# linhthi/BLISS-GNN

Measured on AMD Instinct MI355X. Metric: steps/sec (train step: sample_blocks + gather + SAGE fwd/bwd + Adam + exp3), reddit-like, higher is better.
Workload: dtype bf16

## Files before the change

bliss_gnn_amd/_lib.py:

```python
import ctypes as C
import os

_HERE = os.path.dirname(os.path.abspath(__file__))
LIB_PATH = os.path.join(_HERE, "libbliss_gnn.so")

EINVAL = -1
MODE_BANDIT, MODE_LADIES, MODE_UNIFORM_NODES, MODE_PARTIALS = 0, 1, 4, 8

ERR_BITS = {
    1: "frontier larger than 2^31-1 edges",
    2: "candidate capacity exceeded / seed id out of range",
    4: "kept-node capacity exceeded",
    8: "block-edge capacity exceeded",
    16: "non-finite or negative weight reached an exact reduction",
    32: "exact sum left its fixed-point range",
    64: "seed capacity exceeded",
    128: "random stream ran short / generator made no progress",
    256: "a cross-stream flag never came (bliss_flag_wait timed out)",
}


class Graph(C.Structure):
    _fields_ = [("indptr", C.c_void_p), ("indices", C.c_void_p), ("eid", C.c_void_p),
                ("num_nodes", C.c_int32), ("num_edges", C.c_int64)]


class NodeMaps(C.Structure):
    _fields_ = [("local_id", C.c_void_p), ("first_pos", C.c_void_p), ("acc_p2", C.c_void_p)]


class LayerCounts(C.Structure):
    _fields_ = [("S", C.c_int32), ("E", C.c_int32), ("C", C.c_int32), ("K", C.c_int32), ("B", C.c_int32),
                ("err", C.c_int32), ("iters", C.c_int32), ("all_one", C.c_int32), ("c", C.c_double)]


class LayerWs(C.Structure):
    _fields_ = [("counts", C.c_void_p), ("seg_ptr", C.c_void_p), ("seed_acc", C.c_void_p), ("chunk_cnt", C.c_void_p),
                ("cand_nid", C.c_void_p), ("p", C.c_void_p), ("P", C.c_void_p), ("new_id", C.c_void_p),
                ("kept_nid", C.c_void_p), ("node_prob", C.c_void_p), ("hist", C.c_void_p), ("src_cnt", C.c_void_p), ("cap_c", C.c_int32), ("cap_k", C.c_int32),
                ("n_bins", C.c_int32), ("bin_cap", C.c_int64), ("bin_cursor", C.c_void_p), ("bin_rec", C.c_void_p),
                ("bitmap", C.c_void_p), ("word_prefix", C.c_void_p), ("touched_key", C.c_void_p), ("touched_sum", C.c_void_p),
                ("span_seg", C.c_void_p), ("kept_rec", C.c_void_p), ("span_cnt", C.c_void_p), ("kept_rec_positions", C.c_int64),
                ("kept_map", C.c_void_p), ("entry_flag", C.c_void_p),
                ("fs_ticket", C.c_void_p), ("fs_fanout", C.c_int32), ("fs_is_last", C.c_int32), ("fs_rng_cap", C.c_int32),
                ("fs_reserved", C.c_int32), ("fs_eps", C.c_double), ("fs_rng_ctl", C.c_void_p), ("fs_layer_off", C.c_void_p),
                ("block_ready_flag", C.c_void_p)]


class Exp3Block(C.Structure):
    _fields_ = [("w_pos", C.c_void_p), ("row_sum", C.c_void_p), ("scratch", C.c_void_p), ("norm_out", C.c_void_p),
                ("blk_indptr", C.c_void_p), ("blk_src", C.c_void_p), ("blk_dst", C.c_void_p), ("blk_pos", C.c_void_p),
                ("q_ij", C.c_void_p), ("node_prob", C.c_void_p), ("embed_norm", C.c_void_p), ("alpha_or_null", C.c_void_p),
                ("dst_nid", C.c_void_p), ("n_edges_dev", C.c_void_p), ("rewards_out", C.c_void_p), ("edges_bound", C.c_int32)]


EXP3_MAX_BLOCKS = 8


class Exp3RankLists(C.Structure):
    _fields_ = [("w_pos", C.c_void_p * EXP3_MAX_BLOCKS), ("row_sum", C.c_void_p * EXP3_MAX_BLOCKS),
                ("pos_off_words", C.c_int32 * EXP3_MAX_BLOCKS), ("factor_off_bf16", C.c_int32 * EXP3_MAX_BLOCKS),
                ("count_off_words", C.c_int32 * EXP3_MAX_BLOCKS), ("bound", C.c_int32 * EXP3_MAX_BLOCKS),
                ("n_blocks", C.c_int32), ("n_ranks", C.c_int32), ("rank_stride_words", C.c_int64)]


class PackLists(C.Structure):
    _fields_ = [("pos", C.c_void_p * EXP3_MAX_BLOCKS), ("n_dev", C.c_void_p * EXP3_MAX_BLOCKS),
                ("pos_off_words", C.c_int32 * EXP3_MAX_BLOCKS), ("count_off_words", C.c_int32 * EXP3_MAX_BLOCKS),
                ("bound", C.c_int32 * EXP3_MAX_BLOCKS), ("n_blocks", C.c_int32)]


class TileGemm(C.Structure):
    _fields_ = [("a1", C.c_void_p), ("a1_stride", C.c_int64), ("ids", C.c_void_p),
                ("w1", C.c_void_p), ("w1_stride", C.c_int64), ("k1", C.c_int32),
                ("a2", C.c_void_p), ("a2_stride", C.c_int64), ("w2", C.c_void_p), ("w2_stride", C.c_int64), ("k2", C.c_int32),
                ("bias", C.c_void_p), ("m_bound", C.c_int32), ("m_dev", C.c_void_p), ("n", C.c_int32),
                ("out", C.c_void_p), ("out_stride", C.c_int64), ("a_copy", C.c_void_p), ("copy_stride", C.c_int64),
                ("in_norm", C.c_void_p), ("out_norm", C.c_void_p),
                ("relu", C.c_int32), ("drop_p", C.c_float), ("drop_seed", C.c_uint32), ("drop_ctr", C.c_void_p)]


class DGrad(C.Structure):
    _fields_ = [("a1", C.c_void_p), ("a1_stride", C.c_int64), ("w1", C.c_void_p), ("w1_stride", C.c_int64), ("k1", C.c_int32),
                ("a2", C.c_void_p), ("a2_stride", C.c_int64), ("w2", C.c_void_p), ("w2_stride", C.c_int64), ("k2", C.c_int32),
                ("m2_bound", C.c_int32), ("m2_dev", C.c_void_p),
                ("m_bound", C.c_int32), ("m_dev", C.c_void_p), ("n", C.c_int32), ("out", C.c_void_p), ("out_stride", C.c_int64)]


class WGrad(C.Structure):
    _fields_ = [("d", C.c_void_p), ("d_stride", C.c_int64), ("n_out", C.c_int32),
                ("x", C.c_void_p), ("x_stride", C.c_int64), ("k_in", C.c_int32),
                ("rows_bound", C.c_int32), ("rows_dev", C.c_void_p),
                ("dw", C.c_void_p), ("dw_stride", C.c_int64), ("db", C.c_void_p)]


class GatFused(C.Structure):
    _fields_ = [("indptr", C.c_void_p), ("src", C.c_void_p), ("n_dst", C.c_int32), ("n_dst_dev", C.c_void_p),
                ("feat", C.c_void_p), ("feat_stride", C.c_int64), ("attn", C.c_void_p), ("heads", C.c_int32), ("head_dim", C.c_int32),
                ("negative_slope", C.c_float), ("e", C.c_void_p), ("a", C.c_void_p), ("a_drop", C.c_void_p),
                ("rst", C.c_void_p), ("rst_stride", C.c_int64),
                ("drop_p", C.c_float), ("drop_seed", C.c_uint32), ("drop_ctr", C.c_void_p), ("drop_ctr_used", C.c_void_p),
                ("g", C.c_void_p), ("g_stride", C.c_int64), ("de", C.c_void_p), ("d_er", C.c_void_p), ("d_er_stride", C.c_int64),
                ("dattn_part", C.c_void_p),
                ("wg_row", C.c_void_p), ("n_wg_dev", C.c_void_p), ("cap_wg", C.c_int32), ("row_ws", C.c_void_p), ("seg_part", C.c_void_p),
                ("err", C.c_void_p)]


ADAM_MAX_TENSORS = 32


class AdamTensors(C.Structure):
    _fields_ = [("param", C.c_void_p * ADAM_MAX_TENSORS), ("grad", C.c_void_p * ADAM_MAX_TENSORS),
                ("exp_avg", C.c_void_p * ADAM_MAX_TENSORS), ("exp_avg_sq", C.c_void_p * ADAM_MAX_TENSORS),
                ("numel", C.c_int64 * ADAM_MAX_TENSORS), ("count", C.c_int32)]


class BlockOut(C.Structure):
    _fields_ = [("indptr", C.c_void_p), ("src", C.c_void_p), ("dst", C.c_void_p), ("pos", C.c_void_p),
                ("eid", C.c_void_p), ("edge_weights", C.c_void_p), ("q_ij", C.c_void_p), ("t_indptr", C.c_void_p),
                ("t_edge", C.c_void_p), ("t_scratch", C.c_void_p), ("cap_b", C.c_int32)]


_P, _I32, _I64, _F, _D = C.c_void_p, C.c_int32, C.c_int64, C.c_float, C.c_double

SIGNATURES = {
    "bliss_layer_counts_bytes": [],
    "bliss_frontier_prob": [C.POINTER(Graph), C.POINTER(NodeMaps), _P, _P, _I32, _P, _I32, C.c_int, _F, _F, _I64, C.POINTER(LayerWs), _P],
    "bliss_rng_stream_begin": [_P, _P, _P, _P, _I32, _P],
    "bliss_rng_stream_wait": [_P, _P, _P, C.c_int, _I32, _P],
    "bliss_rng_stream_end": [_P, _P, _P, _I32, _P, _P],
    "bliss_rng_stream_chain": [_P, _P, _P, _P, _I32, _P, _I32, _P, _P],
    "bliss_rng_stream_ready": [_P],
    "bliss_rng_prepare": [_I32, _P],
    "bliss_mt_jump_poly": [_I64, _P],
    "bliss_flag_wait": [_P, _P, _P],
    "bliss_flag_set_spin_bound": [C.c_int64],
    "bliss_flag_raise": [_P, _P],
    "bliss_gather_rows": [_P, _I64, _P, _I32, _I32, _P, _I64, _P, _P],
    "bliss_exp3_apply_ranks": [C.POINTER(Exp3RankLists), _P, _P, _P, _P],
    "bliss_pack_lists": [C.POINTER(PackLists), _P, _P],
    "bliss_mt19937_uniform": [_P, _P, _I32, _P, _I32, _P],
    "bliss_poisson_select": [C.POINTER(LayerWs), _I32, _D, _P, _P, _P, C.c_int, _I32, _I64, _P],
    "bliss_multinomial_select": [C.POINTER(LayerWs), _P, _I32, _P],
    "bliss_tile_gemm": [C.POINTER(TileGemm), C.POINTER(TileGemm), _P],
    "bliss_cross_entropy": [_P, _I64, _P, _I32, _I32, _P, _P, _I64, _P, _P, _P, _P],
    "bliss_cross_entropy_sum": [_P, _I64, _P, _I64, _P, _P, _I32, _I32, _P, _P, _I64, _P, _P, _P, _P],
    "bliss_cross_entropy_masked": [_P, _I64, _P, _I64, _P, _I32, _P, _I32, _I32, _P, _F, _I32, _P, _P, _I64, _P, _P, _P, _P],
    "bliss_bce_logits": [_P, _I64, _P, _I32, _I32, _P, _P, _I64, _P, _P, _P, _P],
    "bliss_bce_logits_sum": [_P, _I64, _P, _I64, _P, _P, _I32, _I32, _P, _P, _I64, _P, _P, _P, _P],
    "bliss_bce_logits_masked": [_P, _I64, _P, _I64, _P, _I32, _P, _I32, _I32, _P, _F, _I32, _P, _P, _I64, _P, _P, _P, _P],
    "bliss_adam_step": [C.POINTER(AdamTensors), _P, _F, _F, _F, _F, _P],
    "bliss_cand_importance": [_P, _I32, C.c_int, _P, _P, _P],
    "bliss_poisson_scale": [_P, _P, _I32, _D, _P, _P],
    "bliss_keyed_select": [_P, _P, _P, _I32, _P, C.c_uint64, C.c_uint64, _I32, _P, _P, _P],
    "bliss_exp3_normalize_global": [_P, _I64, _P, _P, _P, _P, _P],
    "bliss_build_block": [C.POINTER(Graph), C.POINTER(NodeMaps), _P, _P, _I32, C.c_int, _F, _F, _I64, C.POINTER(LayerWs), C.POINTER(BlockOut), _P],
    "bliss_normalized_edata": [C.POINTER(Graph), _P, _P],
    "bliss_embed_norm": [_P, _I32, _I32, _I64, _P, _P],
    "bliss_spmm_fwd": [_P, _P, _P, _P, _P, _I64, _I32, _P, _I32, _I32, C.c_int, _P, _I64, C.c_int, _P, _P],
    "bliss_spmm_bwd": [_P, _P, _P, _P, _P, _P, _P, _I64, _I32, _P, _I32, _I32, C.c_int, _P, _I64, C.c_int, _P, _P],
    "bliss_block_transpose": [_P, _P, _I32, _I32, _I32, _P, _P, _P, _I64, _P],
    "bliss_spmm_chunk_edges": [_I32],
    "bliss_sage_epilogue_fwd": [_P, _I64, _P, _I64, _I32, _I32, _F, C.c_uint32, _P, _P, _I64, _P, _P],
    "bliss_sage_epilogue_bwd": [_P, _I64, _P, _I64, _I32, _I32, _F, _P, _I64, _P],
    "bliss_gat_chunk_edges": [],
    "bliss_graph_prepare": [_P, _P, _I64, _I32, C.c_int, _P, _P, _P, _P, _P, _P, _I64, _P],
    "bliss_exp3_update": [C.POINTER(Graph), _P, _P, _P, _P, _P, _P, _P, _P, _P, _P, _P, _P, _I32, _P, _I32, _F, _P, _P, C.c_int, _P, _P],
    "bliss_exp3_step": [C.POINTER(Graph), _P, C.POINTER(Exp3Block), _I32, _F, _P, _P],
    "bliss_exp3_normalize_global_rows": [C.POINTER(Exp3Block), _I32, _I64, _P, _I64, _P],
    "bliss_exp3_update_blocks": [C.POINTER(Graph), _P, C.POINTER(Exp3Block), _I32, _F, _P, _P],
    "bliss_exp3_apply": [_P, _P, _P, _P, _P, _I32, _P, _P],
    "bliss_exp3_normalize": [_P, _I64, _P, _P, _P, _P],
    "bliss_row_sum": [_P, _I64, _P, _P],
    "bliss_gat_logits": [_P, _P, _P, _I32, _P, _I64, _P, _I32, _I32, _F, _P, _P],
    "bliss_sage_dgrad": [C.POINTER(DGrad), _P],
    "bliss_sage_wgrad": [C.POINTER(WGrad), _I32, _P, _I64, _P],
    "bliss_shard_local_seeds": [_P, _I32, _P, _I32, _I32, _I32, _P, _P, _P, _P, _P, _P],
    "bliss_shard_scatter_partials": [_P, _P, _P, _P, _P, _P, _P, _I32, _P, _P],
    "bliss_shard_zero_dense": [_P, _I32, _P],
    "bliss_shard_pack_rows": [_P, _P, _I32, _I32, _I32, _P, _I64, _I32, _P, _I64, _P],
    "bliss_shard_place_rows": [_P, _I64, _P, _P, _I32, _P, _I64, _I32, _I32, _P],
    "bliss_shard_take_rows": [_P, _I32, _I64, _I32, _P, _P, _I32, _P, _I64, _I32, _P],
    "bliss_shard_candidates": [_P, _I32, _I32, _P, _P, _P, _P, _P, _I32, _P, _P, _P],
    "bliss_shard_select_kept": [_P, _P, _P, _P, C.c_uint64, _P, _I32, _P, _I32, _P, _P, _P, _P, _P, _I32, _I32, _I32, _P, _P, _P, _I32, _P, _P, _P],
    "bliss_gat_fused_supported": [_I32, _I32],
    "bliss_gat_segment_edges": [],
    "bliss_gat_fused_stamps": [_P, _P],
    "bliss_gat_segments": [_P, _I32, _I32, _P, _P, _P, _P],
    "bliss_gat_fused_fwd": [C.POINTER(GatFused), _P],
    "bliss_gat_fused_bwd_dst": [C.POINTER(GatFused), _P, _P, _P, _P],
    "bliss_gat_rows_src_fused": [_P, _I32, _P, _P, _P, _P, _I32, _P, _P, _P, _I64, _P, _I64, _P, _I32, _I32, _F, _P, _I64, _P, _P],
    "bliss_gat_logits_f32": [_P, _P, _P, _I32, _P, _I64, _P, _I32, _I32, _F, _P, _P],
    "bliss_gat_edge_dot": [_P, _P, _P, _I32, _P, _I64, _P, _I64, _I32, _I32, _P, _P],
    "bliss_gat_edge_softmax": [_P, _I32, _P, _P, _I32, C.c_int, _P, _P],
    "bliss_gat_rows": [C.c_int, _P, _I32, _P, _P, _P, _P, _I32, _P, _P, _I64, _P, _I32, _I32, _F, _P, _I64, _P, _P, _P],
    "bliss_gat_alpha": [_P, _I32, _P, _P, _P, _P, _P],
    "bliss_prof_enable": [C.c_int],
    "bliss_prof_reset": [],
    "bliss_prof_read": [C.c_int, C.POINTER(C.c_double), C.POINTER(C.c_int64)],
    "bliss_prof_kernel_count": [],
}


SPECIAL_SIGNATURES = ("bliss_prof_kernel_name", "bliss_block_transpose_temp_bytes", "bliss_graph_prepare_capacity",
                      "bliss_graph_prepare_temp_bytes", "bliss_rng_stream_handle", "bliss_sage_wgrad_workspace")


def _load():
    if not os.path.exists(LIB_PATH):
        raise ImportError(
            f"{LIB_PATH} not found: build it with `python -c 'import __graft_entry__ as g; g.build()'` "
            "or `make -C bliss_gnn_amd/csrc`.  bliss_gnn_amd has no CPU or PyTorch fallback.")
    lib = C.CDLL(LIB_PATH)
    for name, argtypes in SIGNATURES.items():
        fn = getattr(lib, name)
        fn.argtypes = argtypes
        fn.restype = C.c_int
    lib.bliss_block_transpose_temp_bytes.argtypes = [_I32, _I32]
    lib.bliss_block_transpose_temp_bytes.restype = C.c_int64
    lib.bliss_sage_wgrad_workspace.argtypes = [C.POINTER(WGrad), _I32]
    lib.bliss_sage_wgrad_workspace.restype = C.c_int64
    for name in ("bliss_graph_prepare_capacity", "bliss_graph_prepare_temp_bytes"):
        getattr(lib, name).argtypes = [_I64, _I32, C.c_int]
        getattr(lib, name).restype = C.c_int64
    lib.bliss_rng_stream_handle.argtypes = []
    lib.bliss_rng_stream_handle.restype = C.c_int64
    lib.bliss_prof_kernel_name.argtypes = [C.c_int]
    lib.bliss_prof_kernel_name.restype = C.c_char_p
    assert lib.bliss_layer_counts_bytes() == C.sizeof(LayerCounts), "LayerCounts layout mismatch"
    return lib


lib = _load()


def check(rc, what):
    if rc != 0:
        raise RuntimeError(f"{what} failed with code {rc}" + (" (invalid argument)" if rc == EINVAL else " (hipError_t)"))


def err_string(bits):
    return "; ".join(msg for b, msg in ERR_BITS.items() if bits & b) or "unknown"
```

bliss_gnn_amd/csrc/sage.hip:

```cpp
#include "common.cuh"
#include "bliss_gnn.h"
#include <cstdlib>

namespace {

typedef __bf16 bf16x8_t __attribute__((ext_vector_type(8)));
typedef float f32x16_t __attribute__((ext_vector_type(16)));

#define TG_TPB 512
#define TG_M 32
#define TG_WAVES (TG_TPB / 64)
#define TG_NB (256 / 32 / TG_WAVES)

struct TileGemm {
  const bf16_t* a1; long long a1_stride; const int* ids;
  const bf16_t* w1; long long w1_stride; int k1;
  const bf16_t* a2; long long a2_stride; const bf16_t* w2; long long w2_stride; int k2;
  const bf16_t* bias;
  int m_bound; const int* m_dev; int n;
  bf16_t* out; long long out_stride;
  bf16_t* a_copy; long long copy_stride;
  bf16_t* in_norm; bf16_t* out_norm;
  int relu; unsigned drop_thresh; float drop_scale; unsigned seed; unsigned long long* ctr;
};
// ... 43 lines not shown
    for (int c = lane; c < dim; c += 64)
#pragma unroll
      for (int q = 0; q < RPW; ++q) { const float a = bf2f(tile[(size_t)(q * TG_WAVES + wave) * stride + c]); s[q] += a * a; }
  }
  for (int d = 32; d >= 1; d >>= 1)
#pragma unroll
    for (int q = 0; q < RPW; ++q) s[q] += __shfl_xor(s[q], d);
#pragma unroll
  for (int q = 0; q < RPW; ++q) {
    const int r = row0 + q * TG_WAVES + wave;
    if (lane == 0 && r < m_bound) out[r] = r < M ? f2bf(sqrtf(s[q])) : (bf16_t)0;
  }
}

__device__ __forceinline__ void stage_rows(const bf16_t* __restrict__ a, long long a_stride, const int* row_id, int k,
                                           int row0, int m_bound, bf16_t* tile, int stride, bf16_t* __restrict__ copy, long long copy_stride,
                                           int wave, int lane) {
  const int kp = k_pad16(k);
  const bool even = (k % 2 == 0) && (a_stride % 2 == 0) && (((uintptr_t)a) % 4 == 0);
  const bool copy32 = copy && (copy_stride % 2 == 0) && (((uintptr_t)copy) % 4 == 0);
  if (even) {
    const int dw = k / 2;
    constexpr int MAXC = (1024 / 2 + 63) / 64;
    constexpr int RPW = TG_M / TG_WAVES, HALF = RPW;
#pragma unroll
    for (int hb = 0; hb < 1; ++hb) {
      uint32_t v[HALF][MAXC];
#pragma unroll
      for (int q = 0; q < HALF; ++q) {
        const int id = row_id[(hb * HALF + q) * TG_WAVES + wave];
        const uint32_t* src = reinterpret_cast<const uint32_t*>(a + (long long)(id < 0 ? 0 : id) * a_stride);
#pragma unroll
        for (int j = 0; j < MAXC; ++j) {
          const int c = lane + 64 * j;
          const uint32_t x = src[c < dw ? c : dw - 1];
          v[q][j] = (id >= 0 && c < dw) ? x : 0u;
        }
      }
#pragma unroll
      for (int q = 0; q < HALF; ++q) {
        const int lr = (hb * HALF + q) * TG_WAVES + wave, r = row0 + lr;
        uint32_t* sh = reinterpret_cast<uint32_t*>(tile + (size_t)lr * stride);
#pragma unroll
        for (int j = 0; j < MAXC; ++j) {
          const int c = lane + 64 * j;
          if (c < kp / 2) sh[c] = v[q][j];
          if (copy && r < m_bound && c < dw) {
            if (copy32) reinterpret_cast<uint32_t*>(copy + (long long)r * copy_stride)[c] = v[q][j];
            else { bf16_t* cp = copy + (long long)r * copy_stride + 2 * c; cp[0] = (bf16_t)(v[q][j] & 0xffffu); cp[1] = (bf16_t)(v[q][j] >> 16); }
          }
        }
      }
    }
  } else {
    for (int rd = 0; rd < TG_M / TG_WAVES; ++rd) {
      const int lr = rd * TG_WAVES + wave, r = row0 + lr, id = row_id[lr];
      const bf16_t* src = a + (long long)(id < 0 ? 0 : id) * a_stride;
      bf16_t* sh = tile + (size_t)lr * stride;
      for (int c = lane; c < kp; c += 64) {
        const bf16_t x = (id >= 0 && c < k) ? src[c] : (bf16_t)0;
        sh[c] = x;
        if (copy && r < m_bound && c < k) copy[(long long)r * copy_stride + c] = x;
      }
    }
  }
}

#define TG_SLAB 64
#define TG_WSTRIDE (TG_SLAB + 8)
#define TG_WROWS 256
typedef uint32_t u32x4_a4 __attribute__((ext_vector_type(4), aligned(4)));

struct WRegs { uint4 v[TG_WROWS * TG_SLAB / 8 / TG_TPB]; };

__device__ __forceinline__ void w_slab_load_full(WRegs& g, const bf16_t* __restrict__ w, long long w_stride, int N, int slab, int tid) {
  const int part = tid & 7, k = slab * TG_SLAB + 8 * part;
#pragma unroll
  for (int i = 0; i < (int)(sizeof(g.v) / sizeof(g.v[0])); ++i) {
    int n = i * (TG_TPB / 8) + (tid >> 3);
    n = n < N ? n : N - 1;
    const u32x4_a4 q = *reinterpret_cast<const u32x4_a4*>(w + (long long)n * w_stride + k);
    g.v[i] = make_uint4(q[0], q[1], q[2], q[3]);
  }
}
__device__ __forceinline__ void w_slab_load_tail(WRegs& g, const bf16_t* __restrict__ w, long long w_stride, int N, int K, int slab, int tid) {
  const int part = tid & 7, k = slab * TG_SLAB + 8 * part;
  for (int i = 0; i < (int)(sizeof(g.v) / sizeof(g.v[0])); ++i) {
    int n = i * (TG_TPB / 8) + (tid >> 3);
    n = n < N ? n : N - 1;
    const bf16_t* p = w + (long long)n * w_stride + k;
    union { uint4 u; bf16_t e[8]; } t;
    t.u = make_uint4(0, 0, 0, 0);
    for (int j = 0; j < 8; ++j) if (k + j < K) t.e[j] = p[j];
    g.v[i] = t.u;
  }
}
__device__ __forceinline__ int w_full_slabs(const bf16_t* w, long long w_stride, int K) {
  return ((w_stride % 2 == 0) && (((uintptr_t)w) % 4 == 0)) ? K / TG_SLAB : 0;
}
__device__ __forceinline__ void w_slab_store(const WRegs& g, bf16_t* wl, int tid) {
  const int part = tid & 7;
#pragma unroll
  for (int i = 0; i < (int)(sizeof(g.v) / sizeof(g.v[0])); ++i) {
    const int n = i * (TG_TPB / 8) + (tid >> 3);
    *reinterpret_cast<uint4*>(wl + (size_t)n * TG_WSTRIDE + 8 * part) = g.v[i];
  }
}

__device__ __forceinline__ void mma_product(WRegs& ga, WRegs& gb, const bf16_t* tile, int stride, int k, const bf16_t* __restrict__ w,
                                            long long w_stride, int n0, int N, bf16_t* wl, int tid, int lane, f32x16_t acc[TG_NB]) {
  const int kp = k_pad16(k), r = lane & 31, h = lane >> 5;
  const int nslab = (kp + TG_SLAB - 1) / TG_SLAB;
  auto multiply = [&](int sl) {
    if (n0 < N) {
#pragma unroll
      for (int st = 0; st < TG_SLAB / 16; ++st) {
        const int ks = sl * TG_SLAB + 16 * st;
        if (ks < kp) {
          const bf16x8_t a = *reinterpret_cast<const bf16x8_t*>(tile + (size_t)r * stride + ks + 8 * h);
#pragma unroll
          for (int nb = 0; nb < TG_NB; ++nb) {
            const bf16x8_t b = *reinterpret_cast<const bf16x8_t*>(wl + (size_t)(n0 + 32 * nb + r) * TG_WSTRIDE + 16 * st + 8 * h);
            acc[nb] = __builtin_amdgcn_mfma_f32_32x32x16_bf16(a, b, acc[nb], 0, 0, 0);
          }
        }
      }
    }
  };
  const int nfull = w_full_slabs(w, w_stride, k);
  for (int sl = 0; sl < nfull; sl += 2) {
    __syncthreads();
    w_slab_store(ga, wl, tid);
    if (sl + 2 < nfull) w_slab_load_full(ga, w, w_stride, N, sl + 2, tid);
    __syncthreads();
    multiply(sl);
    if (sl + 1 < nfull) {
      __syncthreads();
      w_slab_store(gb, wl, tid);
      if (sl + 3 < nfull) w_slab_load_full(gb, w, w_stride, N, sl + 3, tid);
      __syncthreads();
      multiply(sl + 1);
    }
  }
  for (int sl = nfull; sl < nslab; ++sl) {
    WRegs t;
    w_slab_load_tail(t, w, w_stride, N, k, sl, tid);
    __syncthreads();
    w_slab_store(t, wl, tid);
    __syncthreads();
    multiply(sl);
  }
}

__device__ __forceinline__ void tile_gemm_body(const TileGemm& p, bf16_t* lds, int* row_id, int dbg) {
  const int tid = threadIdx.x, wave = tid >> 6, lane = tid & 63;
  int M = p.m_bound;
  if (p.m_dev) { const int t = *p.m_dev; M = t < M ? t : M; }
  const int row0 = blockIdx.x * TG_M;
  const uint32_t ctr = p.drop_thresh ? (uint32_t)__hip_atomic_load(p.ctr, __ATOMIC_RELAXED, __HIP_MEMORY_SCOPE_AGENT) : 0u;
  const int N = p.n;
  if (row0 >= p.m_bound) return;
  if (row0 >= M) {
    for (int lr = wave; lr < TG_M; lr += TG_WAVES) {
      const int r = row0 + lr;
      if (r >= p.m_bound) break;
      for (int c = lane; c < N; c += 64) p.out[(long long)r * p.out_stride + c] = 0;
      if (p.a_copy) for (int c = lane; c < p.k1; c += 64) p.a_copy[(long long)r * p.copy_stride + c] = 0;
      if (lane == 0) { if (p.in_norm) p.in_norm[r] = 0; if (p.out_norm) p.out_norm[r] = 0; }
    }
    return;
  }
  const int s1 = lds_stride(p.k1), s2 = p.k2 ? lds_stride(p.k2) : 0;
  bf16_t* t1 = lds;
  bf16_t* t2 = lds + (size_t)TG_M * s1;
  const int n0 = wave * 32 * TG_NB;
  bf16_t* wl = lds + (size_t)TG_M * (s1 + s2);
  float bias_v[TG_NB];
#pragma unroll
  for (int nb = 0; nb < TG_NB; ++nb) bias_v[nb] = 0.f;
#pragma unroll
  for (int nb = 0; nb < TG_NB; ++nb) { const int col = n0 + 32 * nb + (lane & 31); if (p.bias && col < N) bias_v[nb] = bf2f(p.bias[col]); }
  WRegs ga, gb;
  {
    const int nf = w_full_slabs(p.w1, p.w1_stride, p.k1);
    if (nf > 0) w_slab_load_full(ga, p.w1, p.w1_stride, N, 0, tid);
    if (nf > 1) w_slab_load_full(gb, p.w1, p.w1_stride, N, 1, tid);
  }
  if (tid < TG_M) {
    const int r = row0 + tid;
    row_id[tid] = r < M ? (p.ids ? p.ids[r] : r) : -1;
    row_id[TG_M + tid] = r < M ? r : -1;
  }
  __syncthreads();
  if (!(dbg & 1)) stage_rows(p.a1, p.a1_stride, row_id, p.k1, row0, p.m_bound, t1, s1, p.a_copy, p.copy_stride, wave, lane);
  if (p.k2) stage_rows(p.a2, p.a2_stride, row_id + TG_M, p.k2, row0, p.m_bound, t2, s2, nullptr, 0, wave, lane);
  __syncthreads();
  if (p.in_norm && !(dbg & 4)) rows_norm(t1, s1, p.k1, row0, M, p.m_bound, p.in_norm, wave, lane);
  f32x16_t acc[TG_NB];
#pragma unroll
  for (int m = 0; m < TG_NB; ++m)
#pragma unroll
    for (int i = 0; i < 16; ++i) acc[m][i] = 0.f;
  if (!(dbg & 2)) mma_product(ga, gb, t1, s1, p.k1, p.w1, p.w1_stride, n0, N, wl, tid, lane, acc);
  if (p.k2) {
    const int nf = w_full_slabs(p.w2, p.w2_stride, p.k2);
    if (nf > 0) w_slab_load_full(ga, p.w2, p.w2_stride, N, 0, tid);
    if (nf > 1) w_slab_load_full(gb, p.w2, p.w2_stride, N, 1, tid);
    mma_product(ga, gb, t2, s2, p.k2, p.w2, p.w2_stride, n0, N, wl, tid, lane, acc);
  }
  __syncthreads();
  const int so = ((N + 63) & ~63) + 8;
  bf16_t* ot = lds;
  if (n0 < N) {
#pragma unroll
    for (int m = 0; m < TG_NB; ++m) {
      const int col = n0 + 32 * m + (lane & 31);
      const float bv = bias_v[m];
#pragma unroll
      for (int i = 0; i < 16; ++i) {
        const int lr = (i & 3) + 8 * (i >> 2) + 4 * (lane >> 5);
        float t = rbf(acc[m][i] + bv);
        if (p.relu) t = t > 0.f ? t : 0.f;
        if (p.drop_thresh) {
          const bool keep = tg_drop_hash(p.seed, ctr, (uint32_t)((row0 + lr) * N + col)) >= p.drop_thresh;
          t = keep ? rbf(t * p.drop_scale) : 0.f;
        }
        ot[(size_t)lr * so + col] = (row0 + lr < M && col < N) ? f2bf(t) : (bf16_t)0;
      }
    }
  }
  __syncthreads();
  const bool pair_ok = (N % 2 == 0) && (p.out_stride % 2 == 0) && (((uintptr_t)p.out) % 4 == 0);
  for (int lr = wave; lr < TG_M; lr += TG_WAVES) {
    const int r = row0 + lr;
    if (r >= p.m_bound) break;
    const bf16_t* sh = ot + (size_t)lr * so;
    bf16_t* o = p.out + (long long)r * p.out_stride;
    if (pair_ok) for (int c = lane * 2; c < N; c += 128) *reinterpret_cast<uint32_t*>(o + c) = *reinterpret_cast<const uint32_t*>(sh + c);
    else for (int c = lane; c < N; c += 64) o[c] = sh[c];
  }
  if (p.out_norm) rows_norm(ot, so, N, row0, M, p.m_bound, p.out_norm, wave, lane);
}

__global__ void __launch_bounds__(TG_TPB) k_tile_gemm(TileGemm p0, TileGemm p1, int n_sets, int dbg) {
  extern __shared__ __attribute__((aligned(16))) bf16_t tg_lds[];
  __shared__ int row_id[2 * TG_M];
  if (dbg & 8) return;
  tile_gemm_body(blockIdx.y == 0 ? p0 : p1, tg_lds, row_id, dbg);
  unsigned long long* ctr = p0.drop_thresh ? p0.ctr : (n_sets > 1 && p1.drop_thresh ? p1.ctr : nullptr);
  if (ctr) {
    __syncthreads();
    if (threadIdx.x == 0) {
      const unsigned long long total = (unsigned long long)gridDim.x * gridDim.y;
      if (atomicAdd(ctr + 1, 1ull) == total - 1) {
        __hip_atomic_store(ctr + 1, 0ull, __ATOMIC_RELAXED, __HIP_MEMORY_SCOPE_AGENT);
        atomicAdd(ctr, 1ull);
      }
    }
  }
}

bool convert(const bliss_tile_gemm_t* a, TileGemm* p, size_t* lds_bytes, int* tiles) {
  if (!a->a1 || !a->w1 || !a->out || a->k1 <= 0 || a->k1 > 1024 || a->n <= 0 || a->n > 256 || a->m_bound <= 0) return false;
  if (a->k2 < 0 || a->k2 > 1024 || (a->k2 > 0 && (!a->a2 || !a->w2))) return false;
  if (a->drop_p < 0.f || a->drop_p >= 1.f || (a->drop_p > 0.f && !a->drop_ctr)) return false;
  p->a1 = (const bf16_t*)a->a1; p->a1_stride = a->a1_stride; p->ids = a->ids;
  p->w1 = (const bf16_t*)a->w1; p->w1_stride = a->w1_stride; p->k1 = a->k1;
  p->a2 = (const bf16_t*)a->a2; p->a2_stride = a->a2_stride; p->w2 = (const bf16_t*)a->w2; p->w2_stride = a->w2_stride; p->k2 = a->k2;
  p->bias = (const bf16_t*)a->bias; p->m_bound = a->m_bound; p->m_dev = a->m_dev; p->n = a->n;
  p->out = (bf16_t*)a->out; p->out_stride = a->out_stride; p->a_copy = (bf16_t*)a->a_copy; p->copy_stride = a->copy_stride;
  p->in_norm = (bf16_t*)a->in_norm; p->out_norm = (bf16_t*)a->out_norm; p->relu = a->relu;
  p->drop_thresh = a->drop_p > 0.f ? (unsigned)((double)a->drop_p * 4294967296.0) : 0u;
  p->drop_scale = a->drop_p > 0.f ? 1.0f / (1.0f - a->drop_p) : 1.0f;
  p->seed = a->drop_seed; p->ctr = (unsigned long long*)a->drop_ctr;
  const size_t stage = ((size_t)TG_M * (lds_stride(a->k1) + (a->k2 ? lds_stride(a->k2) : 0)) + (size_t)TG_WROWS * TG_WSTRIDE) * sizeof(bf16_t);
  const size_t outt = (size_t)TG_M * (((a->n + 63) & ~63) + 8) * sizeof(bf16_t);
  *lds_bytes = stage > outt ? stage : outt;
  *tiles = (a->m_bound + TG_M - 1) / TG_M;
  return true;
}

}

extern "C" int bliss_tile_gemm(const bliss_tile_gemm_t* first, const bliss_tile_gemm_t* second, void* stream) {
  if (!first) return BLISS_EINVAL;
  TileGemm p0, p1;
  size_t l0 = 0, l1 = 0;
  int t0 = 0, t1 = 0;
  if (!convert(first, &p0, &l0, &t0)) return BLISS_EINVAL;
  p1 = p0;
  if (second && !convert(second, &p1, &l1, &t1)) return BLISS_EINVAL;
  const size_t lds = l0 > l1 ? l0 : l1;
  if (lds > 160 * 1024) return BLISS_EINVAL;
  static size_t lds_set = 0;
  if (lds > lds_set) {
    if (hipFuncSetAttribute((const void*)k_tile_gemm, hipFuncAttributeMaxDynamicSharedMemorySize, (int)lds) != hipSuccess) return BLISS_EINVAL;
    lds_set = lds;
  }
  const dim3 grid(t0 > t1 ? t0 : t1, second ? 2 : 1);
  static const int dbg = []() { const char* e = getenv("BLISS_TG_DEBUG"); return e ? atoi(e) : 0; }();
  k_tile_gemm<<<grid, TG_TPB, lds, (hipStream_t)stream>>>(p0, p1, second ? 2 : 1, dbg);
  return (int)hipGetLastError();
}
```

include/bliss_gnn.h:

```cpp
#ifndef BLISS_GNN_H
#define BLISS_GNN_H
#include <stdint.h>

#ifdef __cplusplus
extern "C" {
#endif

#define BLISS_EINVAL (-1)

#define BLISS_MODE_BANDIT 0
#define BLISS_MODE_LADIES 1
#define BLISS_ROWSUM_SLOTS 32
#define BLISS_NORM_SCRATCH (2 + 3 * BLISS_ROWSUM_SLOTS)
#define BLISS_MODE_UNIFORM_NODES 4
#define BLISS_MODE_PARTIALS 8

typedef struct {
  const int64_t* indptr;
  const int32_t* indices;
  const int32_t* eid;
  int32_t num_nodes;
  int64_t num_edges;
} bliss_graph_t;

typedef struct {
  int32_t* local_id;
  uint32_t* first_pos;
  uint64_t* acc_p2;
} bliss_node_maps_t;

typedef struct {
  int32_t S, E, C, K, B;
  int32_t err;
  int32_t iters;
  int32_t all_one;
  double c;
} bliss_layer_counts_t;

typedef struct {
  void* counts;
  int32_t* seg_ptr;
  void* seed_acc;
  int32_t* chunk_cnt;
  int32_t* cand_nid;
  void* p;
  void* P;
  int32_t* new_id;
  int32_t* kept_nid;
  void* node_prob;
  int32_t* hist;
  int32_t* src_cnt;
  int32_t cap_c, cap_k;
  int32_t n_bins;
  int64_t bin_cap;
  int32_t* bin_cursor;
  uint64_t* bin_rec;
  uint32_t* bitmap;
  int32_t* word_prefix;
  uint64_t* touched_key;
  uint64_t* touched_sum;
  int32_t* span_seg;
  void* kept_rec;
  int32_t* span_cnt;
  int64_t kept_rec_positions;
  int32_t* kept_map;
  int32_t* entry_flag;
  int32_t* fs_ticket; int32_t fs_fanout, fs_is_last, fs_rng_cap, fs_reserved; double fs_eps; int32_t* fs_rng_ctl; int32_t* fs_layer_off;
  int32_t* block_ready_flag;
} bliss_layer_ws_t;

typedef struct {
  int32_t* indptr;
  int32_t* src;
  int32_t* dst;
  int32_t* pos;
  int32_t* eid;
  void* edge_weights;
  void* q_ij;
  int32_t* t_indptr;
  int32_t* t_edge;
  int32_t* t_scratch;
  int32_t cap_b;
} bliss_block_out_t;

int bliss_layer_counts_bytes(void);

int bliss_flag_wait(int32_t* flag, int32_t* err_word, void* stream);
int bliss_flag_set_spin_bound(int64_t spins);
int bliss_flag_raise(int32_t* flag, void* stream);

int bliss_frontier_prob(const bliss_graph_t* g, const bliss_node_maps_t* maps, const void* w_pos,
                        const int32_t* seeds, int32_t n_seeds, const int32_t* n_seeds_dev, int32_t cap_s, int mode,
                        float eta_f, float one_minus_eta_f, int64_t frontier_bound, const bliss_layer_ws_t* ws,
                        void* stream);

int bliss_poisson_select(const bliss_layer_ws_t* ws, int32_t fanout, double eps, const float* uniforms,
                         int32_t* uniforms_offset_dev, int32_t* rng_ctl, int is_last, int32_t rng_cap_total,
                         int64_t cand_bound, void* stream);

int bliss_multinomial_select(const bliss_layer_ws_t* ws, const int32_t* chosen, int32_t n_chosen, void* stream);

int bliss_build_block(const bliss_graph_t* g, const bliss_node_maps_t* maps, const void* w_pos,
                      const int32_t* seeds, int32_t cap_s, int mode, float eta_f, float one_minus_eta_f,
                      int64_t frontier_bound, const bliss_layer_ws_t* ws, const bliss_block_out_t* out, void* stream);

int bliss_mt19937_uniform(void* state, const int32_t* n_dev, int32_t n_word_offset, float* out, int32_t cap, void* stream);

int bliss_rng_stream_begin(const void* state, int32_t* ctl, float* out, uint32_t* raw, int32_t cap_total, void* stream);
int bliss_rng_prepare(int32_t cap_total, int32_t* plan4);
int bliss_mt_jump_poly(int64_t n_words, uint32_t* poly_words);
int bliss_rng_stream_wait(int32_t* ctl, const void* counts, int32_t* layer_off, int is_last, int32_t cap_total, void* stream);
int bliss_rng_stream_end(void* state, const int32_t* ctl, const uint32_t* raw, int32_t cap_total, int32_t* err_word,
                         void* stream);
int bliss_rng_stream_chain(void* state, int32_t* ctl, float* out, uint32_t* raw, int32_t cap_total, int32_t* counts_dev,
                           int32_t n_count_words, int32_t* counts_host, void* stream);
int bliss_rng_stream_ready(void* stream);
int64_t bliss_rng_stream_handle(void);

int bliss_cand_importance(const int64_t* sums, int32_t n, int uniform_nodes, void* p_bf16, int32_t* err, void* stream);
int bliss_poisson_scale(int32_t* hist, void* counts, int32_t fanout, double eps, int32_t* scratch, void* stream);
int bliss_keyed_select(const int32_t* nid, const void* p_bf16, const uint8_t* is_seed, int32_t n, const void* counts,
                       uint64_t seed, uint64_t step, int32_t layer, void* P_bf16, uint8_t* keep, void* stream);
int bliss_shard_local_seeds(const int32_t* seeds_g, int32_t n_seeds, const int32_t* n_seeds_dev, int32_t lo, int32_t hi, int32_t cap_s,
                            int32_t* seeds_l, int32_t* seeds_l_copy, int32_t* seed_pos, int32_t* n_local_dev, int32_t* err, void* stream);
int bliss_shard_scatter_partials(const int32_t* seeds_l, const int64_t* seed_p2, const int32_t* n_local_dev, const int64_t* touched_key,
                                 const int64_t* touched_sum, const int32_t* n_touched_dev, int64_t* dense, int32_t num_nodes,
                                 int32_t* err, void* stream);
int bliss_shard_pack_rows(const int32_t* nid, const int32_t* n_rows_dev, int32_t cap_rows, int32_t lo, int32_t hi, const void* table_bf16,
                          int64_t table_stride, int32_t row_len, void* out_bf16, int64_t out_stride, void* stream);
int bliss_shard_place_rows(const void* src_bf16, int64_t src_stride, const int32_t* pos, const int32_t* n_dev, int32_t cap_s, void* out_bf16,
                           int64_t out_stride, int32_t n_rows, int32_t row_len, void* stream);
int bliss_shard_take_rows(const void* src, int32_t src_is_f32, int64_t src_stride, int32_t n_src_rows, const int32_t* pos, const int32_t* n_dev,
                          int32_t cap_s, void* out_bf16, int64_t out_stride, int32_t row_len, void* stream);
int bliss_shard_zero_dense(int64_t* dense, int32_t num_nodes, void* stream);
int bliss_shard_candidates(int64_t* dense, int32_t num_nodes, int32_t uniform_nodes, int32_t* cand_nid, void* p_bf16, uint8_t* is_seed,
                           int32_t* hist, void* counts, int32_t cap_c, int32_t* scratch, int32_t* err, void* stream);
int bliss_shard_select_kept(const int32_t* cand_nid, const void* p_bf16, const uint8_t* is_seed, const void* counts, uint64_t seed,
                            int64_t* step_dev, int32_t layer, const int32_t* seeds_g, int32_t n_seeds, const int32_t* n_seeds_dev,
                            void* P_bf16, int32_t* kept_nid, void* node_prob_bf16, int32_t* kept_map, int32_t cap_k, int32_t cap_c,
                            int32_t num_nodes, void* layer_counts, const int32_t* n_local_dev, int32_t* scratch, int32_t bump_step,
                            int32_t* done_flag, int32_t* err, void* stream);
int bliss_exp3_normalize_global(void* w_pos, int64_t num_edges, int64_t* row_sum, const int64_t* norm_limbs, int64_t* scratch,
                                void* norm_out_bf16, void* stream);

typedef struct {
  const void* a1; int64_t a1_stride; const int32_t* ids;
  const void* w1; int64_t w1_stride; int32_t k1;
  const void* a2; int64_t a2_stride; const void* w2; int64_t w2_stride; int32_t k2;
  const void* bias;
  int32_t m_bound; const int32_t* m_dev; int32_t n;
  void* out; int64_t out_stride;
  void* a_copy; int64_t copy_stride;
  void* in_norm; void* out_norm;
  int32_t relu; float drop_p; uint32_t drop_seed; void* drop_ctr;
} bliss_tile_gemm_t;
int bliss_tile_gemm(const bliss_tile_gemm_t* first, const bliss_tile_gemm_t* second_or_null, void* stream);

typedef struct {
  const void* a1; int64_t a1_stride; const void* w1; int64_t w1_stride; int32_t k1;
  const void* a2; int64_t a2_stride; const void* w2; int64_t w2_stride; int32_t k2; int32_t m2_bound; const int32_t* m2_dev;
  int32_t m_bound; const int32_t* m_dev; int32_t n;
  void* out; int64_t out_stride;
} bliss_dgrad_t;
int bliss_sage_dgrad(const bliss_dgrad_t* args, void* stream);
typedef struct {
  const void* d; int64_t d_stride; int32_t n_out;
  const void* x; int64_t x_stride; int32_t k_in;
  int32_t rows_bound; const int32_t* rows_dev;
  void* dw; int64_t dw_stride; void* db;
} bliss_wgrad_t;
int64_t bliss_sage_wgrad_workspace(const bliss_wgrad_t* probs, int32_t n_probs);
int bliss_sage_wgrad(const bliss_wgrad_t* probs, int32_t n_probs, float* partials, int64_t partial_floats, void* stream);

int bliss_cross_entropy(const void* logits, int64_t stride, const int64_t* labels, int32_t n_rows, int32_t n_cls,
                        float* row_loss, void* dlogits, int64_t d_stride, float* loss_out, uint32_t* ticket, int32_t* err,
                        void* stream);
int bliss_cross_entropy_sum(const void* logits, int64_t stride, const void* logits2, int64_t stride2, const int64_t* label_table,
                            const int32_t* label_ids, int32_t n_rows, int32_t n_cls, float* row_loss, void* dlogits, int64_t d_stride,
                            float* loss_out, uint32_t* ticket, int32_t* err, void* stream);
int bliss_cross_entropy_masked(const void* logits, int64_t stride, const void* logits2, int64_t stride2, const int64_t* label_table,
                               int32_t n_table, const int32_t* label_ids, int32_t id_off, int32_t n_rows, const int32_t* n_rows_dev,
                               float denom, int32_t n_cls, float* row_loss, void* dlogits, int64_t d_stride, float* loss_out,
                               uint32_t* ticket, int32_t* err, void* stream);

int bliss_bce_logits(const void* logits, int64_t stride, const float* targets, int32_t n_rows, int32_t n_cls, float* row_loss,
                     void* dlogits, int64_t d_stride, float* loss_out, uint32_t* ticket, int32_t* err, void* stream);
int bliss_bce_logits_sum(const void* logits, int64_t stride, const void* logits2, int64_t stride2, const float* target_table,
                         const int32_t* label_ids, int32_t n_rows, int32_t n_cls, float* row_loss, void* dlogits, int64_t d_stride,
                         float* loss_out, uint32_t* ticket, int32_t* err, void* stream);
int bliss_bce_logits_masked(const void* logits, int64_t stride, const void* logits2, int64_t stride2, const float* target_table,
                            int32_t n_table, const int32_t* label_ids, int32_t id_off, int32_t n_rows, const int32_t* n_rows_dev,
                            float denom, int32_t n_cls, float* row_loss, void* dlogits, int64_t d_stride, float* loss_out,
                            uint32_t* ticket, int32_t* err, void* stream);

#define BLISS_ADAM_MAX_TENSORS 32
typedef struct {
  void* param[BLISS_ADAM_MAX_TENSORS];
  const void* grad[BLISS_ADAM_MAX_TENSORS];
  void* exp_avg[BLISS_ADAM_MAX_TENSORS];
  void* exp_avg_sq[BLISS_ADAM_MAX_TENSORS];
  int64_t numel[BLISS_ADAM_MAX_TENSORS];
  int32_t count;
} bliss_adam_t;
int bliss_adam_step(const bliss_adam_t* tensors, float* state, float beta1, float beta2, float eps, float weight_decay, void* stream);

int bliss_normalized_edata(const bliss_graph_t* g, void* w_pos, void* stream);

int bliss_gather_rows(const void* feat, int64_t feat_stride, const int32_t* ids, int32_t n_rows, int32_t dim, void* out,
                      int64_t out_stride, void* norm_out, void* stream);

int bliss_embed_norm(const void* h, int32_t n_rows, int32_t dim, int64_t row_stride, void* out, void* stream);

int bliss_spmm_chunk_edges(int32_t nnz_bound);
int bliss_spmm_fwd(const int32_t* indptr, const int32_t* src, const int32_t* dst, const void* w, const void* h,
                   int64_t h_stride, int32_t n_dst, const int32_t* nnz_dev, int32_t nnz, int32_t dim, int mean, void* out,
                   int64_t out_stride, int out_fp32, float* partials, void* stream);

int bliss_spmm_bwd(const int32_t* t_indptr, const int32_t* t_edge, const int32_t* src, const int32_t* dst,
                   const int32_t* indptr, const void* w, const void* gout, int64_t gout_stride, int32_t n_src,
                   const int32_t* nnz_dev, int32_t nnz, int32_t dim, int mean, void* gh, int64_t gh_stride, int out_fp32,
                   float* partials, void* stream);

int bliss_sage_epilogue_fwd(const void* a, int64_t a_stride, const void* b, int64_t b_stride, int32_t n_rows, int32_t dim,
                            float p_drop, uint32_t seed, uint64_t* ctr, void* out, int64_t out_stride, void* norm_out, void* stream);
int bliss_sage_epilogue_bwd(const void* dout, int64_t dout_stride, const void* out, int64_t out_stride, int32_t n_rows, int32_t dim,
                            float p_drop, void* din, int64_t din_stride, void* stream);

int64_t bliss_block_transpose_temp_bytes(int32_t cap_b, int32_t n_src_cap);
int bliss_block_transpose(const int32_t* src, const int32_t* nnz_dev, int32_t nnz, int32_t cap_b, int32_t n_src_cap,
                          int32_t* t_indptr, int32_t* t_edge, void* temp, int64_t temp_bytes, void* stream);

int64_t bliss_graph_prepare_capacity(int64_t n_edges, int32_t num_nodes, int undirected);
int64_t bliss_graph_prepare_temp_bytes(int64_t n_edges, int32_t num_nodes, int undirected);
int bliss_graph_prepare(const int32_t* coo_src, const int32_t* coo_dst, int64_t n_edges, int32_t num_nodes, int undirected,
                        int64_t* indptr, int32_t* indices, int32_t* eid, int64_t* n_out, int32_t* err, void* temp,
                        int64_t temp_bytes, void* stream);

int bliss_exp3_update(const bliss_graph_t* g, const void* edge_w_pos, void* w_pos, int64_t* row_sum,
                      const int32_t* blk_indptr, const int32_t* blk_src, const int32_t* blk_dst,
                      const int32_t* blk_pos, const void* q_ij, const void* node_prob, const void* embed_norm,
                      const void* alpha_or_null, const int32_t* dst_nid, int32_t n_dst, const int32_t* n_edges_dev,
                      int32_t edges_bound, float delta_f, void* rewards_out, void* factor_out, int apply,
                      int32_t* err, void* stream);

#define BLISS_EXP3_MAX_BLOCKS 8
typedef struct {
  void* w_pos; int64_t* row_sum; int64_t* scratch; void* norm_out;
  const int32_t *blk_indptr, *blk_src, *blk_dst, *blk_pos;
  const void *q_ij, *node_prob, *embed_norm, *alpha_or_null;
  const int32_t* dst_nid; const int32_t* n_edges_dev;
  void* rewards_out;
  int32_t edges_bound;
} bliss_exp3_block_t;
int bliss_exp3_step(const bliss_graph_t* g, const void* edge_w_pos, const bliss_exp3_block_t* blocks, int32_t n_blocks,
                    float delta_f, int32_t* err, void* stream);
int bliss_exp3_update_blocks(const bliss_graph_t* g, const void* edge_w_pos, const bliss_exp3_block_t* blocks, int32_t n_blocks,
                             float delta_f, int32_t* err, void* stream);
int bliss_exp3_normalize_global_rows(const bliss_exp3_block_t* rows, int32_t n_rows, int64_t num_edges, const int64_t* norm_limbs,
                                     int64_t limb_stride, void* stream);

int bliss_exp3_apply(void* w_pos, int64_t* row_sum, const int32_t* pos, const void* factor, const int32_t* n_dev,
                     int32_t n_bound, int32_t* err, void* stream);

typedef struct {
  void* w_pos[BLISS_EXP3_MAX_BLOCKS];
  int64_t* row_sum[BLISS_EXP3_MAX_BLOCKS];
  int32_t pos_off_words[BLISS_EXP3_MAX_BLOCKS], factor_off_bf16[BLISS_EXP3_MAX_BLOCKS], count_off_words[BLISS_EXP3_MAX_BLOCKS],
      bound[BLISS_EXP3_MAX_BLOCKS];
  int32_t n_blocks, n_ranks;
  int64_t rank_stride_words;
} bliss_exp3_rank_lists_t;
int bliss_exp3_apply_ranks(const bliss_exp3_rank_lists_t* lists, const int32_t* gathered, int32_t* barrier, int32_t* err, void* stream);

typedef struct {
  const int32_t* pos[BLISS_EXP3_MAX_BLOCKS];
  const int32_t* n_dev[BLISS_EXP3_MAX_BLOCKS];
  int32_t pos_off_words[BLISS_EXP3_MAX_BLOCKS], count_off_words[BLISS_EXP3_MAX_BLOCKS], bound[BLISS_EXP3_MAX_BLOCKS];
  int32_t n_blocks;
} bliss_pack_lists_t;
int bliss_pack_lists(const bliss_pack_lists_t* lists, int32_t* buf, void* stream);

int bliss_exp3_normalize(void* w_pos, int64_t num_edges, int64_t* row_sum, int64_t* scratch, void* norm_out_bf16,
                         void* stream);

int bliss_row_sum(const void* w_pos, int64_t num_edges, int64_t* row_sum, void* stream);

int bliss_gat_chunk_edges(void);
int bliss_gat_logits(const int32_t* src, const int32_t* dst, const int32_t* nnz_dev, int32_t nnz, const void* feat,
                     int64_t feat_stride, const void* attn, int32_t heads, int32_t head_dim, float negative_slope, void* e_out,
                     void* stream);
typedef struct {
  const int32_t* indptr; const int32_t* src; int32_t n_dst; const int32_t* n_dst_dev;
  const void* feat; int64_t feat_stride; const void* attn; int32_t heads; int32_t head_dim; float negative_slope;
  void* e; void* a; void* a_drop;
  void* rst; int64_t rst_stride;
  float drop_p; uint32_t drop_seed; void* drop_ctr; void* drop_ctr_used;
  const void* g; int64_t g_stride; void* de; void* d_er; int64_t d_er_stride; float* dattn_part;
  const int32_t* wg_row; const int32_t* n_wg_dev; int32_t cap_wg; void* row_ws; float* seg_part; int32_t* err;
} bliss_gat_fused_t;
int bliss_gat_segment_edges(void);
int bliss_gat_fused_stamps(long long* stamps, long long* stamps_bwd);
int bliss_gat_segments(const int32_t* indptr, int32_t n_dst, int32_t cap_wg, int32_t* wg_row, int32_t* n_wg_dev, int32_t* err, void* stream);
int bliss_gat_fused_supported(int32_t heads, int32_t head_dim);
int bliss_gat_rows_src_fused(const int32_t* t_indptr, int32_t n_src, const int32_t* t_edge, const int32_t* src, const int32_t* dst,
                             const int32_t* nnz_dev, int32_t nnz, const void* de, const void* a_drop, const void* feat, int64_t feat_stride,
                             const void* g, int64_t g_stride, const void* attn, int32_t heads, int32_t head_dim, float negative_slope,
                             void* out, int64_t out_stride, float* partials, void* stream);
int bliss_gat_fused_fwd(const bliss_gat_fused_t* args, void* stream);
int bliss_gat_fused_bwd_dst(const bliss_gat_fused_t* args, float* block_sums, float* d_attn, uint32_t* ticket, void* stream);
// ... 24 lines not shown
```

Before: 1461.

## Add small-grid tile GEMM variant with per-wave weight loading and wave-local sync

Adds a templated SMALL path for the SAGE tile GEMM, used when the grid has at most 128 workgroups. In this path each wave loads its own 32-column weight slab in batches of four, double-buffered in registers. It orders its LDS accesses with wave-level fences instead of workgroup-wide barriers, and handles both weight operands in one loop. The aim is to cut barrier stalls and serialization in small, latency-bound GEMMs, such as the last sampled layers, at the cost of more registers and redundant per-wave work. An env var can disable it.

```diff
diff --git a/bliss_gnn_amd/_lib.py b/bliss_gnn_amd/_lib.py
--- a/bliss_gnn_amd/_lib.py
+++ b/bliss_gnn_amd/_lib.py
@@ -143,6 +143,7 @@
     "bliss_poisson_select": [C.POINTER(LayerWs), _I32, _D, _P, _P, _P, C.c_int, _I32, _I64, _P],
     "bliss_multinomial_select": [C.POINTER(LayerWs), _P, _I32, _P],
     "bliss_tile_gemm": [C.POINTER(TileGemm), C.POINTER(TileGemm), _P],
+    "bliss_tile_gemm_variant": [_I32, _I32],
     "bliss_cross_entropy": [_P, _I64, _P, _I32, _I32, _P, _P, _I64, _P, _P, _P, _P],
     "bliss_cross_entropy_sum": [_P, _I64, _P, _I64, _P, _P, _I32, _I32, _P, _P, _I64, _P, _P, _P, _P],
     "bliss_cross_entropy_masked": [_P, _I64, _P, _I64, _P, _I32, _P, _I32, _I32, _P, _F, _I32, _P, _P, _I64, _P, _P, _P, _P],
diff --git a/bliss_gnn_amd/csrc/sage.hip b/bliss_gnn_amd/csrc/sage.hip
--- a/bliss_gnn_amd/csrc/sage.hip
+++ b/bliss_gnn_amd/csrc/sage.hip
@@ -219,6 +219,98 @@
   }
 }
 
+#define TG_SMALL_WGS 128
+#define TG_BATCH 4
+struct WBatch { uint4 v[TG_BATCH][4]; };
+
+__device__ __forceinline__ void wave_lds_order() {
+  __builtin_amdgcn_fence(__ATOMIC_RELEASE, "wavefront");
+  __builtin_amdgcn_wave_barrier();
+  __builtin_amdgcn_fence(__ATOMIC_ACQUIRE, "wavefront");
+}
+
+__device__ __forceinline__ void w_own_load(uint4 (&v)[4], const bf16_t* __restrict__ w, long long w_stride, int N, int K, int nfull,
+                                           int slab, int n0, int lane) {
+  const int part = lane & 7, k = slab * TG_SLAB + 8 * part;
+  if (slab < nfull) {
+#pragma unroll
+    for (int i = 0; i < 4; ++i) {
+      int n = n0 + 8 * i + (lane >> 3);
+      n = n < N ? n : N - 1;
+      const u32x4_a4 q = *reinterpret_cast<const u32x4_a4*>(w + (long long)n * w_stride + k);
+      v[i] = make_uint4(q[0], q[1], q[2], q[3]);
+    }
+  } else {
+#pragma unroll
+    for (int i = 0; i < 4; ++i) {
+      int n = n0 + 8 * i + (lane >> 3);
+      n = n < N ? n : N - 1;
+      const bf16_t* p = w + (long long)n * w_stride + k;
+      union { uint4 u; bf16_t e[8]; } t;
+      t.u = make_uint4(0, 0, 0, 0);
+#pragma unroll
+      for (int j = 0; j < 8; ++j) if (k + j < K) t.e[j] = p[j];
+      v[i] = t.u;
+    }
+  }
+}
+
+struct WProd {
+  const bf16_t* w; long long w_stride; int K, kp, nslab, nfull, nb;
+  const bf16_t* tile; int stride;
+};
+__device__ __forceinline__ WProd w_prod(const bf16_t* w, long long w_stride, int K, const bf16_t* tile, int stride) {
+  WProd q;
+  q.w = w; q.w_stride = w_stride; q.K = K; q.kp = k_pad16(K); q.tile = tile; q.stride = stride;
+  q.nslab = K ? (q.kp + TG_SLAB - 1) / TG_SLAB : 0;
+  q.nfull = K ? w_full_slabs(w, w_stride, K) : 0;
+  q.nb = (q.nslab + TG_BATCH - 1) / TG_BATCH;
+  return q;
+}
+struct WSmall { WProd p1, p2; int n0, N, lane; bf16_t* wl; };
+
+__device__ __forceinline__ void ws_load_batch(const WSmall& s, WBatch& g, int b) {
+  const bool second = b >= s.p1.nb;
+  const WProd m = second ? s.p2 : s.p1;
+  const int sl0 = (second ? b - s.p1.nb : b) * TG_BATCH;
+#pragma unroll
+  for (int q = 0; q < TG_BATCH; ++q)
+    if (sl0 + q < m.nslab) w_own_load(g.v[q], m.w, m.w_stride, s.N, m.K, m.nfull, sl0 + q, s.n0, s.lane);
+}
+
+__device__ __forceinline__ void ws_mul_batch(const WSmall& s, const WBatch& g, int b, f32x16_t acc[TG_NB]) {
+  const bool second = b >= s.p1.nb;
+  const WProd m = second ? s.p2 : s.p1;
+  const int sl0 = (second ? b - s.p1.nb : b) * TG_BATCH;
+  const int r = s.lane & 31, h = s.lane >> 5, part = s.lane & 7;
+  const bf16_t* tile = m.tile;
+  const int stride = m.stride, kp = m.kp;
+#pragma unroll
+  for (int q = 0; q < TG_BATCH; ++q) {
+    const int sl = sl0 + q;
+    if (sl < m.nslab) {
+      wave_lds_order();
+#pragma unroll
+      for (int i = 0; i < 4; ++i)
+        *reinterpret_cast<uint4*>(s.wl + (size_t)(s.n0 + 8 * i + (s.lane >> 3)) * TG_WSTRIDE + 8 * part) = g.v[q][i];
+      wave_lds_order();
+#pragma unroll
+      for (int st = 0; st < TG_SLAB / 16; ++st) {
+        const int ks = sl * TG_SLAB + 16 * st;
+        if (ks < kp) {
+          const bf16x8_t a = *reinterpret_cast<const bf16x8_t*>(tile + (size_t)r * stride + ks + 8 * h);
+#pragma unroll
+          for (int nb = 0; nb < TG_NB; ++nb) {
+            const bf16x8_t bb = *reinterpret_cast<const bf16x8_t*>(s.wl + (size_t)(s.n0 + 32 * nb + r) * TG_WSTRIDE + 16 * st + 8 * h);
+            acc[nb] = __builtin_amdgcn_mfma_f32_32x32x16_bf16(a, bb, acc[nb], 0, 0, 0);
+          }
+        }
+      }
+    }
+  }
+}
+
+template <bool SMALL>
 __device__ __forceinline__ void tile_gemm_body(const TileGemm& p, bf16_t* lds, int* row_id, int dbg) {
   const int tid = threadIdx.x, wave = tid >> 6, lane = tid & 63;
   int M = p.m_bound;
@@ -248,7 +340,18 @@
 #pragma unroll
   for (int nb = 0; nb < TG_NB; ++nb) { const int col = n0 + 32 * nb + (lane & 31); if (p.bias && col < N) bias_v[nb] = bf2f(p.bias[col]); }
   WRegs ga, gb;
-  {
+  WBatch ba, bb;
+  WSmall ws;
+  int nbatch = 0;
+  if (SMALL) {
+    static_assert(TG_NB == 1, "a wave owns one 32-column block");
+    ws.p1 = w_prod(p.w1, p.w1_stride, p.k1, t1, s1);
+    ws.p2 = w_prod(p.w2, p.w2_stride, p.k2, t2, s2);
+    ws.n0 = n0; ws.N = N; ws.lane = lane; ws.wl = wl;
+    nbatch = n0 < N ? ws.p1.nb + ws.p2.nb : 0;
+    if (nbatch > 0) ws_load_batch(ws, ba, 0);
+    if (nbatch > 1) ws_load_batch(ws, bb, 1);
+  } else {
     const int nf = w_full_slabs(p.w1, p.w1_stride, p.k1);
     if (nf > 0) w_slab_load_full(ga, p.w1, p.w1_stride, N, 0, tid);
     if (nf > 1) w_slab_load_full(gb, p.w1, p.w1_stride, N, 1, tid);
@@ -268,8 +371,17 @@
   for (int m = 0; m < TG_NB; ++m)
 #pragma unroll
     for (int i = 0; i < 16; ++i) acc[m][i] = 0.f;
-  if (!(dbg & 2)) mma_product(ga, gb, t1, s1, p.k1, p.w1, p.w1_stride, n0, N, wl, tid, lane, acc);
-  if (p.k2) {
+  if (SMALL) {
+    for (int b = 0; b < nbatch; b += 2) {
+      ws_mul_batch(ws, ba, b, acc);
+      if (b + 2 < nbatch) ws_load_batch(ws, ba, b + 2);
+      if (b + 1 < nbatch) {
+        ws_mul_batch(ws, bb, b + 1, acc);
+        if (b + 3 < nbatch) ws_load_batch(ws, bb, b + 3);
+      }
+    }
+  } else if (!(dbg & 2)) mma_product(ga, gb, t1, s1, p.k1, p.w1, p.w1_stride, n0, N, wl, tid, lane, acc);
+  if (!SMALL && p.k2) {
     const int nf = w_full_slabs(p.w2, p.w2_stride, p.k2);
     if (nf > 0) w_slab_load_full(ga, p.w2, p.w2_stride, N, 0, tid);
     if (nf > 1) w_slab_load_full(gb, p.w2, p.w2_stride, N, 1, tid);
@@ -309,11 +421,12 @@
   if (p.out_norm) rows_norm(ot, so, N, row0, M, p.m_bound, p.out_norm, wave, lane);
 }
 
+template <bool SMALL>
 __global__ void __launch_bounds__(TG_TPB) k_tile_gemm(TileGemm p0, TileGemm p1, int n_sets, int dbg) {
   extern __shared__ __attribute__((aligned(16))) bf16_t tg_lds[];
   __shared__ int row_id[2 * TG_M];
   if (dbg & 8) return;
-  tile_gemm_body(blockIdx.y == 0 ? p0 : p1, tg_lds, row_id, dbg);
+  tile_gemm_body<SMALL>(blockIdx.y == 0 ? p0 : p1, tg_lds, row_id, dbg);
   unsigned long long* ctr = p0.drop_thresh ? p0.ctr : (n_sets > 1 && p1.drop_thresh ? p1.ctr : nullptr);
   if (ctr) {
     __syncthreads();
@@ -349,6 +462,14 @@
 
 }
 
+extern "C" int bliss_tile_gemm_variant(int32_t m_bound, int32_t second_m_bound) {
+  if (m_bound <= 0 || second_m_bound < 0) return BLISS_EINVAL;
+  const char* e = getenv("BLISS_TG_SMALL");
+  if (e && e[0] == '0') return 0;
+  const int64_t t0 = ((int64_t)m_bound + TG_M - 1) / TG_M, t1 = ((int64_t)second_m_bound + TG_M - 1) / TG_M;
+  return (t0 > t1 ? t0 : t1) * (second_m_bound ? 2 : 1) <= TG_SMALL_WGS ? 1 : 0;
+}
+
 extern "C" int bliss_tile_gemm(const bliss_tile_gemm_t* first, const bliss_tile_gemm_t* second, void* stream) {
   if (!first) return BLISS_EINVAL;
   TileGemm p0, p1;
@@ -359,13 +480,16 @@
   if (second && !convert(second, &p1, &l1, &t1)) return BLISS_EINVAL;
   const size_t lds = l0 > l1 ? l0 : l1;
   if (lds > 160 * 1024) return BLISS_EINVAL;
-  static size_t lds_set = 0;
-  if (lds > lds_set) {
-    if (hipFuncSetAttribute((const void*)k_tile_gemm, hipFuncAttributeMaxDynamicSharedMemorySize, (int)lds) != hipSuccess) return BLISS_EINVAL;
-    lds_set = lds;
-  }
   const dim3 grid(t0 > t1 ? t0 : t1, second ? 2 : 1);
   static const int dbg = []() { const char* e = getenv("BLISS_TG_DEBUG"); return e ? atoi(e) : 0; }();
-  k_tile_gemm<<<grid, TG_TPB, lds, (hipStream_t)stream>>>(p0, p1, second ? 2 : 1, dbg);
+  const bool small = !dbg && bliss_tile_gemm_variant(first->m_bound, second ? second->m_bound : 0) == 1;
+  static size_t lds_set[2] = {0, 0};
+  if (lds > lds_set[small]) {
+    const void* fn = small ? (const void*)k_tile_gemm<true> : (const void*)k_tile_gemm<false>;
+    if (hipFuncSetAttribute(fn, hipFuncAttributeMaxDynamicSharedMemorySize, (int)lds) != hipSuccess) return BLISS_EINVAL;
+    lds_set[small] = lds;
+  }
+  if (small) k_tile_gemm<true><<<grid, TG_TPB, lds, (hipStream_t)stream>>>(p0, p1, second ? 2 : 1, dbg);
+  else k_tile_gemm<false><<<grid, TG_TPB, lds, (hipStream_t)stream>>>(p0, p1, second ? 2 : 1, dbg);
   return (int)hipGetLastError();
 }
diff --git a/include/bliss_gnn.h b/include/bliss_gnn.h
--- a/include/bliss_gnn.h
+++ b/include/bliss_gnn.h
@@ -155,6 +155,7 @@
   int32_t relu; float drop_p; uint32_t drop_seed; void* drop_ctr;
 } bliss_tile_gemm_t;
 int bliss_tile_gemm(const bliss_tile_gemm_t* first, const bliss_tile_gemm_t* second_or_null, void* stream);
+int bliss_tile_gemm_variant(int32_t m_bound, int32_t second_m_bound);
 
 typedef struct {
   const void* a1; int64_t a1_stride; const void* w1; int64_t w1_stride; int32_t k1;
```

Result: no change. 1465, median of 2 (+0.3%).
